# ash-shar/Long-Tail-GAN

Measured on AMD Instinct MI355X. Metric: train users/sec at BATCH_SIZE=100, higher is better.
Workload: dtype bf16

## Files before the change

### long-tail-gan_amd/csrc/ltg_fast_gen.h

```cpp
#pragma once


typedef LtgRg<1, 2, 1, 1, 4> Rg16x32;
typedef LtgRg<1, 2, 1, 1, 8> Rg16x32k8;
struct LtgRaw2 {
    ltg_f32x4 x, y;
};
constexpr int ENC1_NT = 512;
template <bool PRE>
__global__ __launch_bounds__(ENC1_NT) void fk_enc1(int B, int H, int Z, const float* __restrict__ h1, const float* __restrict__ Wq1,
                                              const float* __restrict__ bq1, const float* __restrict__ eps_in, float is_training,
                                              uint64_t seed, uint64_t step, float* __restrict__ mulv, float* __restrict__ z,
                                              const float* __restrict__ bq0 = nullptr, float* __restrict__ h1_out = nullptr,
                                              LtgGate end_wait = LTG_NO_GATE) {
    LTG_STAMP_AT(11, 0);
    __shared__ __attribute__((aligned(16))) float lds[Rg16x32k8::LDS_FLOATS];
    const LtgTile2 tl = xcd_tile2();
    const int m0 = tl.y * 16, n0 = tl.x * 16, Z2 = 2 * Z;
    auto col = [=] __device__(int c) { return min(n0 + (c & 15), Z - 1) + (c >> 4) * Z; };
    auto a_ld = [=] __device__(int, int m, int k) {
        if constexpr (PRE) return LtgRaw2{ltg_ld4(h1 + (size_t)m * H + k), ltg_ld4(bq0 + k)};
        else return ltg_ld4(h1 + (size_t)m * H + k);
    };
    const bool keep_h1 = PRE && tl.x == 0;
// ... 123 lines not shown
                                            float anneal, uint64_t seed, uint64_t step, float* __restrict__ dmlv) {
    LTG_STAMP_AT(15, 0);
    __shared__ __attribute__((aligned(16))) float lds[Rg16::LDS_FLOATS];
    const LtgTile2 tl = xcd_tile2();
    dz_tile(B, Z, H, da2, Wp0, mulv, eps_in, is_training, anneal, seed, step, dmlv, tl.y * 16, tl.x * 16, lds);
}
__global__ __launch_bounds__(NT) void fk_dz_dh2(int B, int Z, int H, const float* __restrict__ dh2, const float* __restrict__ h2,
                                                const float* __restrict__ Wp0, const float* __restrict__ mulv, const float* __restrict__ eps_in,
                                                float is_training, float anneal, uint64_t seed, uint64_t step, float* __restrict__ dmlv,
                                                float* __restrict__ da2_out) {
    __shared__ __attribute__((aligned(16))) float lds[Rg16::LDS_FLOATS];
    const LtgTile2 tl = xcd_tile2();
    dz_tile<true>(B, Z, H, dh2, Wp0, mulv, eps_in, is_training, anneal, seed, step, dmlv, tl.y * 16, tl.x * 16, lds, h2, da2_out, tl.x == 0);
}
__global__ __launch_bounds__(NT) void fk_dh1(int B, int H, int Z2, const float* __restrict__ dmlv, const float* __restrict__ Wq1,
                                             const float* __restrict__ h1, float* __restrict__ da1) {
    LTG_STAMP_AT(16, 0);
    __shared__ __attribute__((aligned(16))) float lds[Rg16::LDS_FLOATS];
    const LtgTile2 tl = xcd_tile2();
    dh1_tile(B, H, Z2, dmlv, Wq1, h1, da1, tl.y * 16, tl.x * 16, lds);
}

constexpr int E0_U = 8;
__global__ __launch_bounds__(ENC_NT) void fk_enc0_fwd(int H, int I, const int32_t* __restrict__ indptr, const int32_t* __restrict__ indices,
                                                      const float* __restrict__ values, const uint8_t* __restrict__ drop_keep, float keep,
                                                      uint64_t seed, uint64_t step, const float* __restrict__ Wq0,
                                                      const float* __restrict__ bq0, float* __restrict__ h1, float* __restrict__ row_scale,
                                                      const float* __restrict__ row_norm2, int item_lo, int Ig, int pre_only,
                                                      float* __restrict__ xd, int rps, LtgGate started = LTG_NO_GATE, LtgGate end_wait = LTG_NO_GATE) {
    if (end_wait.word && blockIdx.y == gridDim.y - 1) {
        if (blockIdx.x == 0 && threadIdx.x == 0) ltg_gate_wait_tail(end_wait);
        return;
    }
    if (blockIdx.x == 0 && blockIdx.y == 0 && threadIdx.x == 0) ltg_gate_set(started);
    extern __shared__ __attribute__((aligned(16))) float s_row[];
    __shared__ __attribute__((aligned(16))) float4 s_part[ENC_NW][64];
    __shared__ int s_idx[ENC_NT];
    __shared__ float s_val[ENC_NT];
    __shared__ float red[ENC_NW];
    const int b = blockIdx.y, cb = blockIdx.x, tid = threadIdx.x, lane = tid & 63, w = tid >> 6;
    const uint64_t kb = rps > 0 ? (uint64_t)(b % rps) : (uint64_t)b;
    step += rps > 0 ? (uint64_t)(b / rps) : 0;
    const int beg = indptr[b], end = indptr[b + 1];
    float4 bb = make_float4(0.f, 0.f, 0.f, 0.f);
    if (!pre_only && tid < 64 && 64 * cb + tid < (H >> 2)) bb = *reinterpret_cast<const float4*>(bq0 + 4 * (64 * cb + tid));
    float ss = 0.f;
    for (int e = beg + tid; e < end; e += ENC_NT) {
        const float v = values ? values[e] : 1.f;
        ss += v * v;
    }
#pragma unroll
    for (int o = 32; o > 0; o >>= 1) ss += __shfl_xor(ss, o);
    if (lane == 0) red[w] = ss;
    __syncthreads();
    ss = 0.f;
#pragma unroll
    for (int i = 0; i < ENC_NW; ++i) ss += red[i];
    if (row_norm2) ss = row_norm2[b];
    const float scale = 1.f / (keep * sqrtf(fmaxf(ss, 1e-12f)));
    if (tid == 0 && cb == 0) row_scale[b] = scale;
    const int H4 = H >> 2;
    const int c4 = min(64 * cb + lane, H4 - 1);
    const bool dense = xd != nullptr && cb == 0;
// ... 314 lines not shown
```

### long-tail-gan_amd/csrc/ltg_fast_small.h

```cpp
#pragma once


template <bool BF>
__global__ __launch_bounds__(NT) void fk_dec1(int B, int I, int H, const float* __restrict__ h2, const float* __restrict__ Wp1t,
                                              const float* __restrict__ bp1, float* __restrict__ logits) {
    __shared__ __attribute__((aligned(16))) float lds[Rg16::LDS_FLOATS];
    const LtgTile2 tl = xcd_tile2();
    const int m0 = tl.y * 16, n0 = tl.x * 16;
    auto a_ld = [=] __device__(int, int m, int k) { return ltg_ld4(h2 + (size_t)m * H + k); };
    auto b_ld = [=] __device__(int, int k, int n) { return ltg_ld4(Wp1t + (size_t)n * H + k); };
    auto xf = [=] __device__(ltg_f32x4 v, int, int, int) { return BF ? ltg_bf16r4(v) : v; };
    const float biasv = bp1[min(n0 + (int)(threadIdx.x & 15), I - 1)];
    auto epi = [=] __device__(int, int m, int n, float v, bool ok) {
        if (ok) logits[(size_t)m * I + n] = v + biasv;
    };
    if constexpr (BF) ltg_rgemm<1, 1, 1, 1, 4, 5, true>(B, I, H, m0, n0, a_ld, xf, b_ld, xf, epi, lds);
    else ltg_rgemm<1, 1, 1, 1, 4, 10>(B, I, H, m0, n0, a_ld, xf, b_ld, xf, epi, lds);
}

__device__ __forceinline__ void block_red4(float& a, float& b, float& c, float& mx, float (*red)[NT / 64]) {
#pragma unroll
    for (int o = 32; o > 0; o >>= 1) {
        a += __shfl_xor(a, o);
        b += __shfl_xor(b, o);
// ... 120 lines not shown
    const float l = mx + logf(s);
    const float ps = psu / s;
    const float invB = 1.f / (float)B, invs = 1.f / s;
    const float c = cntv > 0 ? lam / (float)cntv * sy : 0.f;
    const float alpha = nx * invB + c * ps;
#pragma unroll
    for (int j = 0; j < PER; ++j) {
        const int i = tid + NT * j;
        if (i < I) {
            const float p = expf(v[j] - mx) * invs;
            dlog[(size_t)b * I + i] = p * alpha - s_x[i] * invB - (s_s[i] ? c * p : 0.f);
        }
    }
    if (tid == 0) {
        lse[b] = l;
        float* o = rowout + (size_t)b * 4;
        o[0] = -xl + nx * l;
        o[1] = ps;
        o[2] = klb;
        o[3] = sy;
    }
}

constexpr int DH2_NT = 512;
template <bool BF>
__global__ __launch_bounds__(DH2_NT) void fk_dh2(int B, int I, int H, const float* __restrict__ dlog, const float* __restrict__ Wp1t,
                                             const float* __restrict__ h2, float* __restrict__ da2) {
    __shared__ __attribute__((aligned(16))) float lds[LtgRg<1, 1, 1, 1, 8>::LDS_FLOATS];
    const LtgTile2 tl = xcd_tile2();
    const int m0 = tl.y * 16, n0 = tl.x * 16;
    auto a_ld = [=] __device__(int, int m, int k) { return ltg_ld4(dlog + (size_t)m * I + k); };
    auto b_ld = [=] __device__(int, int k, int n) { return ltg_ld4s(Wp1t + (size_t)k * H + n, H); };
    auto xf = [=] __device__(ltg_f32x4 v, int, int, int) { return BF ? ltg_bf16r4(v) : v; };
    const float t = h2[(size_t)min(m0 + (int)(threadIdx.x >> 4), B - 1) * H + min(n0 + (int)(threadIdx.x & 15), H - 1)];
    auto epi = [=] __device__(int, int m, int n, float v, bool ok) {
        if (ok) da2[(size_t)m * H + n] = v * (1.f - t * t);
    };
    if constexpr (BF) ltg_rgemm<1, 1, 1, 1, 8, 4, true>(B, H, I, m0, n0, a_ld, xf, b_ld, xf, epi, lds);
    else ltg_rgemm<1, 1, 1, 1, 8, 8>(B, H, I, m0, n0, a_ld, xf, b_ld, xf, epi, lds);
}

struct WgTensors {
    float *W, *mW, *vW, *b, *mb, *vb;
};
struct WgWhere {
    float *p, *m, *v;
    bool vec;
};
struct WgRegs {
    ltg_f32x4 p, m, v;
};
#ifndef LTG_TAIL_BN
#define LTG_TAIL_BN 32
#endif
template <bool RND, bool ONES_L>
__device__ __forceinline__ void wgrad_adam_tile(int K, int Min, int Nin, const float* __restrict__ Lm, int ldl, const float* __restrict__ Rm,
                                                int ldr, WgTensors T, int ldw, AdamC ad, int m0, int n0, float* __restrict__ lds, unsigned dead = 0u) {
    const int M = ONES_L ? Min + 1 : Min, N = ONES_L ? Nin : Nin + 1;
    auto a_ld = [=] __device__(int, int m, int k) {
        ltg_f32x4 v;
#pragma unroll
// ... 225 lines not shown
```

### long-tail-gan_amd/csrc/ltg_gemm.h

```cpp
#pragma once
#include <hip/hip_runtime.h>
#include <stdint.h>

typedef __attribute__((ext_vector_type(4))) float ltg_f32x4;
typedef __attribute__((ext_vector_type(8))) __bf16 ltg_bf16x8;
typedef __attribute__((ext_vector_type(8))) unsigned short ltg_u16x8;

__device__ __forceinline__ unsigned short ltg_f2bf(float x) {
    unsigned u = __float_as_uint(x);
    u += 0x7FFFu + ((u >> 16) & 1u);
    return (unsigned short)(u >> 16);
}

__device__ __forceinline__ unsigned char ltg_f2fp8(float x) {
    const float c = fminf(fmaxf(x, -448.f), 448.f);
    return (unsigned char)(__builtin_amdgcn_cvt_pk_fp8_f32(c, 0.f, 0, false) & 0xFF);
}

template <int MODE, int BK_> struct LtgGemmCfg;
template <int BK_> struct LtgGemmCfg<1, BK_> {
    typedef unsigned short T;
    static constexpr int BK = BK_;
    static constexpr int LDK = BK_ + 8;
    static_assert(BK_ % 32 == 0, "bf16 K-step is 32");
// ... 214 lines not shown
                for (int r = 0; r < 4; ++r)
                    Cs[(wm * WTM + i * 16 + lq * 4 + r) * LDC + wn * WTN + j * 16 + lr] = acc[i][j][r];
        __syncthreads();
        constexpr int N4 = BN / 4;
#pragma unroll
        for (int e = tid; e < BM * N4; e += NT) {
            const int mm = e / N4, c4 = e % N4;
            const int m = m0 + mm, n = n0 + c4 * 4;
            if (m < M && n < N) epi(m, n, *reinterpret_cast<const float4*>(&Cs[mm * LDC + c4 * 4]));
        }
    } else {
#pragma unroll
        for (int i = 0; i < TM; ++i)
#pragma unroll
            for (int j = 0; j < TN; ++j)
#pragma unroll
                for (int r = 0; r < 4; ++r) {
                    const int m = m0 + wm * WTM + i * 16 + lq * 4 + r;
                    const int n = n0 + wn * WTN + j * 16 + lr;
                    if (m < M && n < N) epi(m, n, acc[i][j][r]);
                }
    }
}
```

### long-tail-gan_amd/csrc/ltg_kernels.hip

```cpp
#include <hip/hip_runtime.h>
#include <math.h>
#include <stdint.h>

#include "../../include/ltg.h"
#include "ltg_gemm.h"
#include "ltg_rng.h"

namespace {

constexpr int NT = 256;

struct AdamC {
    float lr_t, b1, b2, eps;
};

__device__ __forceinline__ float adam_move(const float p, const float lm, const float v, const float eps) {
#ifdef LTG_ADAM_IEEE
    return p - lm / (sqrtf(v) + eps);
#else
    return __builtin_fmaf(-lm, __builtin_amdgcn_rcpf(__builtin_amdgcn_sqrtf(v) + eps), p);
#endif
}
__device__ __forceinline__ void adam1(float& p, float& m, float& v, const float g, const float lr_t, const AdamC& c) {
    m = __builtin_fmaf(c.b1, m, (1.f - c.b1) * g);
// ... 121 lines not shown
    return c < 4 * ST_BN ? 4 * ST_BN : c;
}

inline int dh2_kchunk(int I) {
    int chunk = (I + 63) / 64;
    chunk = (chunk + 31) / 32 * 32;
    if (chunk < 256) chunk = 256;
    return chunk;
}

inline size_t gq0_rows(const ltg_config* cfg, int ) { return (size_t)cfg->n_items; }

constexpr int RD_MAXI = 4096;
struct Workspace {
    float *rowpart, *segpart, *nb, *Pb, *scal, *dlog, *part, *dh2, *da2, *dmlv, *da1, *gq0;
    int32_t* slotmap;
    float *A1, *A3, *y, *ds, *lrow, *dpre1, *dpre3, *slab;
    float *spart, *G3, *rowout, *xd;
    uint8_t* A1_8;
    uint8_t *A1T_8, *dpre3_8, *dpre3T_8, *dpre1T_8, *ET_8;
    unsigned short* dA1T_16;
    int np8;
    float* wsp;
    size_t bytes;
};
inline int d_slab_stride(int P) { return (P + 1 + 3) & ~3; }

constexpr int FT_BM = 64, FT_NT = 512;
constexpr int FT_KP1_MAX = 4;
inline int ft_lda(int h12) { return ((h12 + 31) & ~31) + 4; }
inline size_t ft_lds_bytes(int h12) { return ((size_t)FT_BM * ft_lda(h12) + 4 * FT_BM) * sizeof(float); }
inline size_t ft_wsp_triples(int h0, int h1, int h2, int h3) {
    const size_t kp1 = (h0 + 31) / 32, kp3 = (h1 + h2 + 31) / 32;
    return (size_t)((h1 + 15) / 16) * kp1 + (size_t)((h2 + 15) / 16) * kp1 + (size_t)((h3 + 15) / 16) * kp3;
}
inline size_t ft_wsp_bytes(int h0, int h1, int h2, int h3) { return ft_wsp_triples(h0, h1, h2, h3) * 3 * 1024; }
inline bool ft_wsp_capable(const ltg_config* c) {
    return (c->tuning & 262144) == 0 && c->d_precision == LTG_PREC_FP32 && !(c->d_h0 >= 512 && c->d_h1 + c->d_h2 >= 512 && c->d_h3 >= 128) && c->d_h0 >= 4 &&
           c->d_h0 <= 32 * FT_KP1_MAX && (c->d_h0 % 4) == 0 && c->d_h1 >= 1 && c->d_h2 >= 1 && c->d_h3 >= 1 && c->d_h3 <= 320 &&
           ft_lds_bytes(c->d_h1 + c->d_h2) <= (size_t)160 * 1024;
}
Workspace carve(const ltg_config* cfg, int max_rows, int max_pairs, char* base) {
    Workspace w;
    size_t off = 0;
    auto take = [&](size_t nfloat) {
        float* p = reinterpret_cast<float*>(base + off);
        off += align_up(nfloat * sizeof(float));
        return p;
    };
    const size_t R = (size_t)max_rows, I = (size_t)cfg->n_items, H = (size_t)cfg->h_enc, Z = (size_t)cfg->z_dim;
    const size_t P = (size_t)max_pairs, h12 = (size_t)cfg->d_h1 + cfg->d_h2, h3 = (size_t)cfg->d_h3;
    const int kchunk = dh2_kchunk(cfg->n_items);
    size_t nsplit = (I + kchunk - 1) / kchunk;
    {
        const size_t ns2 = (I + dh2_stream_chunk(cfg->n_items) - 1) / dh2_stream_chunk(cfg->n_items);
        if (ns2 > nsplit) nsplit = ns2;
    }
    w.rowpart = take(R * RP);
    w.segpart = take(segpart_floats(I, R));
    w.nb = take(R);
    w.Pb = take(R);
    w.scal = take(16);
    w.dlog = take(R * I);
// ... 14 lines not shown
    {
        const DLayout L = d_layout(cfg->d_h0, cfg->d_h1, cfg->d_h2, cfg->d_h3);
        const size_t ks = (P + D_KCHUNK - 1) / D_KCHUNK;
        w.slab = take(ks * (size_t)d_slab_stride(L.off[8]));
    }
    w.spart = take((((h3 + 31) / 32) + 1) * P);
    w.G3 = take(P * h3);
    w.rowout = take(R * 4);
    w.xd = take(I <= (size_t)RD_MAXI ? R * I : 1);
    w.A1_8 = reinterpret_cast<uint8_t*>(take((P * h12 + 3) / 4));
    {
        const bool f8 = cfg->d_precision == LTG_PREC_FP8;
        const size_t np = ((P + 127) / 128 * 128), h0 = (size_t)cfg->d_h0;
        auto take8 = [&](size_t nbytes) { return reinterpret_cast<uint8_t*>(take(f8 ? (nbytes + 3) / 4 : 1)); };
        w.np8 = (int)np;
        w.A1T_8 = take8((h12 + 1) * np);
        w.dA1T_16 = reinterpret_cast<unsigned short*>(take8(2 * h12 * np));
        w.dpre3_8 = take8(P * h3);
        w.dpre3T_8 = take8(h3 * np);
        w.dpre1T_8 = take8(h12 * np);
        w.ET_8 = take8(2 * (h0 + 1) * np);
    }
    w.wsp = take(ft_wsp_capable(cfg) ? ft_wsp_bytes(cfg->d_h0, cfg->d_h1, cfg->d_h2, cfg->d_h3) / sizeof(float) : 1);
    w.bytes = off;
    return w;
}

inline AdamC make_adam(const ltg_config* cfg, int t) {
    AdamC a;
    const double b1 = cfg->beta1, b2 = cfg->beta2;
    a.lr_t = (float)((double)cfg->lr * sqrt(1.0 - pow(b2, (double)t)) / (1.0 - pow(b1, (double)t)));
    a.b1 = cfg->beta1;
    a.b2 = cfg->beta2;
    a.eps = cfg->adam_eps;
    return a;
}

struct Probe {
    const ltg_probe* p;
    hipStream_t st;
    inline void before(int id) const {
        if (p && p->kernel_id == id && p->ev_start) (void)hipEventRecord((hipEvent_t)p->ev_start, st);
    }
    inline void after(int id) const {
        if (p && p->kernel_id == id && p->ev_stop) (void)hipEventRecord((hipEvent_t)p->ev_stop, st);
    }
// ... 29 lines not shown
}
inline bool d_fast(const ltg_config* c) {
    return fast_on(c) && c->d_precision == LTG_PREC_FP32 && !d_wide(c) && c->d_h3 <= 512 && (c->d_h0 % 4) == 0 && ((c->d_h1 + c->d_h2) % 4) == 0 && (c->d_h3 % 4) == 0;
}
#ifndef LTG_D_SPLIT_SET
#define LTG_D_SPLIT_SET 0xE
#endif
inline int d_spl(const ltg_config* c, int which) {
    const int mode = c->d_arith & 3, set = ((c->d_arith >> 4) & 15) ? ((c->d_arith >> 4) & 15) : (mode == LTG_DARITH_BF16X4 ? 0xF : LTG_D_SPLIT_SET);
    if (mode == LTG_DARITH_FP32 || !((set >> which) & 1)) return 0;
    return mode == LTG_DARITH_BF16X4 ? 4 : 6;
}
#define LTG_D_SPL_LAUNCH(SPLV, KERNEL, ...)                                       \
    do {                                                                          \
        if ((SPLV) == 6) hipLaunchKernelGGL((KERNEL<6>), __VA_ARGS__);            \
        else if ((SPLV) == 4) hipLaunchKernelGGL((KERNEL<4>), __VA_ARGS__);       \
        else hipLaunchKernelGGL((KERNEL<0>), __VA_ARGS__);                        \
    } while (0)
inline bool unsharded(const ltg_config* c) { return c->item_lo == 0 && (c->n_items_global == 0 || c->n_items_global == c->n_items); }
inline bool small_fast(const ltg_config* c, int rows) {
    return fast_on(c) && unsharded(c) && c->n_items <= RD_MAXI && (c->n_items % 4) == 0 && (c->z_dim % 4) == 0 && rows <= 256;
}

constexpr int32_t TUNING_BITS = (1 << 14) | (1 << 17) | (1 << 18) | (1 << 19) | (1 << 20) | (1 << 21) | (1 << 22) | (1 << 26);
bool cfg_ok(const ltg_config* c) {
    return c && c->n_items > 0 && c->h_enc > 0 && c->h_enc <= 768 && (c->h_enc % 4) == 0 && c->z_dim > 0 &&
           c->d_h0 >= 1 && c->d_h1 >= 1 && c->d_h2 >= 1 && c->d_h3 >= 1 &&
           (c->precision == LTG_PREC_BF16 || c->precision == LTG_PREC_FP32) && c->d_precision >= 0 && c->d_precision <= LTG_PREC_FP8 &&
           c->d_arith >= 0 && (c->d_arith & 3) <= LTG_DARITH_BF16X4 && (c->d_arith & ~0xF3) == 0 && (c->tuning & ~TUNING_BITS) == 0;
}

inline int Ig_of(const ltg_config* cfg) { return cfg->n_items_global > 0 ? cfg->n_items_global : cfg->n_items; }

inline bool q0_lazy(const ltg_config* cfg, const ltg_gen_state* gen) {
    return gen->q0_last && gen->q0_lr_hist && gen->q0_period >= 1 && gen->q0_period <= LTG_Q0_HIST / 2 && gen->q0_ord >= 0 && (cfg->h_enc % 4) == 0 &&
           cfg->n_items >= 8192;
}
void q0_touch(const ltg_config* cfg, const ltg_gen_state* gen, const ltg_batch* bt, hipStream_t st, const unsigned* poison = nullptr,
              int32_t* mark = nullptr, unsigned seq = 0u) {
    if (!q0_lazy(cfg, gen) || bt->n_rows <= 0) return;
    const AdamC ad = make_adam(cfg, 1);
    if (bt->uptr && bt->csr_pos) {
        if (bt->n_unique > 0)
            hipLaunchKernelGGL(k_q0_touch_unique, dim3(bt->n_unique), dim3(Q0_NT), 0, st, cfg->h_enc, bt->n_unique, bt->uptr, bt->csr_pos, bt->indices, bt->uitem,
                               gen->q0_ord, *gen, ad, poison, mark, seq);
    } else {
        hipLaunchKernelGGL(k_q0_touch_rows, dim3(bt->n_rows), dim3(Q0_NT), 0, st, cfg->h_enc, bt->n_rows, bt->indptr, bt->indices, gen->q0_ord, *gen, ad);
    }
}

void fwd_stage_enc(const ltg_config* cfg, const ltg_gen_state* gen, const ltg_batch* bt, const ltg_fwd_opts* o,
                   const ltg_gen_acts* acts, int pre_only, hipStream_t st, float* xd = nullptr, bool touched = false,
                   LtgGate started = LTG_NO_GATE, LtgGate end_wait = LTG_NO_GATE) {
    const int R = bt->n_rows, I = cfg->n_items, H = cfg->h_enc;
    const Probe pr{o->probe, st};
    if (!touched) q0_touch(cfg, gen, bt, st);
    if (fast_on(cfg)) {
        LTG_PROBED(pr, LTG_K_ENC0_FWD,
                   hipLaunchKernelGGL(fk_enc0_fwd, dim3((H / 4 + 63) / 64, R + (end_wait.word ? 1 : 0)), dim3(ENC_NT), xd ? (size_t)I * sizeof(float) : 0, st, H, I, bt->indptr,
                                      bt->indices, bt->values, o->drop_keep, o->keep_prob, cfg->seed, o->rng_step, gen->p[0], gen->p[4], acts->h1,
                                      acts->row_scale, bt->row_norm2, cfg->item_lo, Ig_of(cfg), pre_only, xd, o->rows_per_step, started, end_wait));
        return;
    }
    LTG_PROBED(pr, LTG_K_ENC0_FWD,
               hipLaunchKernelGGL(k_enc0_fwd, dim3(R), dim3(ENC_NT), (size_t)ENC_NW * H * sizeof(float), st, H, I, bt->indptr, bt->indices,
                                  bt->values, o->drop_keep, o->keep_prob, cfg->seed, o->rng_step, gen->p[0], gen->p[4], acts->h1,
                                  acts->row_scale, bt->row_norm2, cfg->item_lo, Ig_of(cfg), pre_only, o->rows_per_step));
}

int launch_dec1_fwd_stream(const ltg_config* cfg, const ltg_gen_state* gen, int R, const ltg_gen_acts* acts, float* stat, hipStream_t st) {
    const int I = cfg->n_items, H = cfg->h_enc;
    const int st2_min = (cfg->tuning & (1 << 17)) ? 8192 : ST2_MIN_ITEMS;
    if ((cfg->tuning & (1 << 26)) == 0 && I >= st2_min && (size_t)R * (size_t)I < ((size_t)1 << 30) &&
        (size_t)I * (size_t)(ST_KP * 2) < ((size_t)1 << 32)) {
        const int nt2 = (I + 31) / 32, G2 = nt2 < 256 ? nt2 : 256;
#define LTG_ST2(STATS, NTB) hipLaunchKernelGGL((k_dec1_fwd_stream2<STATS, NTB>), dim3(G2), dim3(ST_NT), (size_t)ST_KS * NTB * 64 * 16, st, R, I, H, acts->h2, gen->wp1t_bf16, gen->p[7], acts->logits, stat)
        if (stat) { if (R <= 112) LTG_ST2(true, 7); else LTG_ST2(true, 8); }
        else { if (R <= 112) LTG_ST2(false, 7); else LTG_ST2(false, 8); }
#undef LTG_ST2
        return G2;
    }
    const int ntiles = (I + ST_BN - 1) / ST_BN, G = ntiles < 256 ? ntiles : 256;
// ... 705 lines not shown
    if (ltg_workspace_bytes(cfg, B, nf) > ws_bytes) return LTG_EWORKSPACE;
    hipStream_t st = (hipStream_t)stream;
    Workspace w = carve(cfg, B, nf, (char*)ws);
    const bool have_y = o->y_pre != nullptr;
    if (have_y) w.y = const_cast<float*>(o->y_pre);
    q0_touch(cfg, gen, bt, st);
    const bool aux_sweep = q0_lazy(cfg, gen) && o->aux_stream && o->ev_fork && o->ev_sweep;
    const bool fork = o->aux_stream && o->ev_fork && o->ev_join && nf > 0 && !have_y;
    if (fork || aux_sweep) {
        hipStream_t aux = (hipStream_t)o->aux_stream;
        if (hipEventRecord((hipEvent_t)o->ev_fork, st) != hipSuccess || hipStreamWaitEvent(aux, (hipEvent_t)o->ev_fork, 0) != hipSuccess)
            return LTG_ELAUNCH;
        if (fork) {
            PairView pv{0, nf, nullptr, nullptr, fake->pop, fake->niche};
            DropView dA{nullptr, o->drop_fake[0], 0, 0}, dB{nullptr, o->drop_fake[1], 0, 0}, dC{nullptr, o->drop_fake[2], 0, 0};
            disc_forward(cfg, disc, pv, dA, dB, dC, o->d_keep_prob, o->d_rng_step, w, false, nullptr, aux);
            if (hipEventRecord((hipEvent_t)o->ev_join, aux) != hipSuccess) return LTG_ELAUNCH;
        }
    }
    ltg_g_opts o_local = *o;
    o_local.fake_done = (o->fake_done & 1) | (aux_sweep ? G_AUX_SWEEP : 0);
    o = &o_local;
    const bool small = small_fast(cfg, B);
    fwd_stage_enc(cfg, gen, bt, &o->fwd, acts, 0, st, small ? w.xd : nullptr, true);
    const int sgroups = fwd_stage_rest(cfg, gen, bt, &o->fwd, acts, 0, st, small ? nullptr : w.segpart);
    if (small) {
        const int I = cfg->n_items, H = cfg->h_enc;
        const Probe pr{o->probe, st};
        if (nf > 0 && !fork && !have_y) {
            PairView pv{0, nf, nullptr, nullptr, fake->pop, fake->niche};
            DropView dA{nullptr, o->drop_fake[0], 0, 0}, dB{nullptr, o->drop_fake[1], 0, 0}, dC{nullptr, o->drop_fake[2], 0, 0};
            disc_forward(cfg, disc, pv, dA, dB, dC, o->d_keep_prob, o->d_rng_step, w, false, o->probe, st);
        }
        if (fork && hipStreamWaitEvent(st, (hipEvent_t)o->ev_join, 0) != hipSuccess) return LTG_ELAUNCH;
        LTG_PROBED(pr, LTG_K_ROW_DLOGITS, hipLaunchKernelGGL(fk_row_dlogits, dim3(B), dim3(NT), 0, st, B, I, bt->indptr, bt->indices, bt->values, acts->logits,
                                                             acts->kl_rows, w.y, nf, o->cnt, o->gan_lambda, fake->row, fake->niche, fake->pop, w.dlog,
                                                             acts->lse, w.rowout));
        pr.before(LTG_K_DH2);
        if (cfg->precision == LTG_PREC_BF16) hipLaunchKernelGGL(fk_dh2<true>, grid2(H, B, 16, 16), dim3(DH2_NT), 0, st, B, I, H, w.dlog, gen->p[3], acts->h2, w.da2);
        else hipLaunchKernelGGL(fk_dh2<false>, grid2(H, B, 16, 16), dim3(DH2_NT), 0, st, B, I, H, w.dlog, gen->p[3], acts->h2, w.da2);
        pr.after(LTG_K_DH2);
        g_chain(cfg, gen, bt, o, acts, w, make_adam(cfg, o->adam_t), nullptr, true, loss_out, st);
        return check_launch();
    }
    g_row_partial(cfg, bt, fake, acts, w.rowpart, st, w.segpart, nullptr, sgroups);
    if (fork && hipStreamWaitEvent(st, (hipEvent_t)o->ev_join, 0) != hipSuccess) return LTG_ELAUNCH;
    int rc = g_stage_bwd_dec(cfg, gen, disc, bt, fake, o, acts, w.rowpart, 1, loss_out, w, w.da2, st, fork || have_y, acts->h2);
    if (rc != LTG_OK) return rc;
    rc = g_stage_bwd_rest(cfg, gen, bt, o, acts, w.da2, w, st, true);
    if (aux_sweep && hipStreamWaitEvent(st, (hipEvent_t)o->ev_sweep, 0) != hipSuccess) return LTG_ELAUNCH;
    return rc;
}

int ltg_g_fwd_enc(const ltg_config* cfg, const ltg_gen_state* gen, const ltg_batch* bt, const ltg_fwd_opts* opts,
                  const ltg_gen_acts* acts, ltg_stream stream) {
    clear_errors();
    if (!g_args_ok(cfg, gen, bt, acts) || !opts) return LTG_EINVAL;
    fwd_stage_enc(cfg, gen, bt, opts, acts, 1, (hipStream_t)stream);
    return check_launch();
}

int ltg_g_fwd_rest(const ltg_config* cfg, const ltg_gen_state* gen, const ltg_batch* bt, const ltg_pairs* fake,
// ... 641 lines not shown
```

### long-tail-gan_amd/csrc/ltg_rgemm.h

```cpp
#pragma once
#include <hip/hip_runtime.h>
#include <stdint.h>

#include "ltg_gemm.h"

__device__ __forceinline__ ltg_f32x4 ltg_ld4(const float* __restrict__ p) { return *reinterpret_cast<const ltg_f32x4*>(p); }
__device__ __forceinline__ ltg_f32x4 ltg_ld4s(const float* __restrict__ p, size_t s) { return ltg_f32x4{p[0], p[s], p[2 * s], p[3 * s]}; }
__device__ __forceinline__ float ltg_bf16r(float x) { return __uint_as_float((unsigned)ltg_f2bf(x) << 16); }
__device__ __forceinline__ ltg_f32x4 ltg_bf16r4(ltg_f32x4 v) { return ltg_f32x4{ltg_bf16r(v[0]), ltg_bf16r(v[1]), ltg_bf16r(v[2]), ltg_bf16r(v[3])}; }

#ifdef LTG_STAMP
__device__ unsigned long long ltg_stamp_buf[16384 * 8];
__device__ __forceinline__ void ltg_stamp(int slot) {
    if (threadIdx.x == 0) {
        const unsigned wg = blockIdx.x + gridDim.x * (blockIdx.y + gridDim.y * blockIdx.z);
        if (wg < 16384u)
            ltg_stamp_buf[wg * 8 + slot] = slot == 6 ? ((unsigned long long)__builtin_amdgcn_s_getreg((4 << 0) | (0 << 6) | (31 << 11)) |
                                                        ((unsigned long long)__builtin_amdgcn_s_getreg((20 << 0) | (0 << 6) | (31 << 11)) << 32))
                                                     : wall_clock64();
    }
}
#define LTG_STAMP_AT(SID, slot) do { if constexpr ((SID) == LTG_STAMP) ltg_stamp(slot); } while (0)
#else
#define LTG_STAMP_AT(SID, slot) do { } while (0)
// ... 176 lines not shown
                    for (int tn = 0; tn < TN; ++tn)
                        acc[tm][tn] = __builtin_amdgcn_mfma_f32_16x16x4f32(av[tm][j], bv[tn][j], acc[tm][tn], 0, 0, 0);
        }
    };
    if constexpr (PEEL) {
        pass(0);
        for (int base = NBLK; base < per; base += NBLK) pass(base);
    } else {
        for (int base = 0; base < per; base += NBLK) pass(base);
    }
    LTG_STAMP_AT(SID, 3);
    float* mine = lds + wk * (G::BM * G::LDC);
#pragma unroll
    for (int tm = 0; tm < TM; ++tm)
#pragma unroll
        for (int tn = 0; tn < TN; ++tn)
#pragma unroll
            for (int x = 0; x < 4; ++x)
                mine[((wm * TM + tm) * 16 + 4 * q + x) * G::LDC + (wn * TN + tn) * 16 + r] = acc[tm][tn][x];
    __syncthreads();
    LTG_STAMP_AT(SID, 4);
}

template <int TM, int TN, int WM, int WN, int WK, int NBLK, bool PEEL = false, class ALD, class AXF, class BLD, class BXF, class MID = LtgNoMid>
__device__ __forceinline__ void ltg_rgemm_product_bf16(int M, int N, int K, int m0, int n0, ALD a_ld, AXF a_xf, BLD b_ld, BXF b_xf, float* __restrict__ lds,
                                                       MID mid = MID()) {
    static_assert(WM * WN * WK == 4 || WM * WN * WK == 8, "4 or 8 waves per workgroup");
    typedef LtgRg<TM, TN, WM, WN, WK> G;
    const int tid = threadIdx.x, lane = tid & 63, w = tid >> 6;
    const int r = lane & 15, q = lane >> 4;
    const int wk = w % WK, wn = (w / WK) % WN, wm = w / (WK * WN);
    const int nblk = (K + 31) >> 5;
    const int per = (nblk + WK - 1) / WK;
    const int Kc = K >= 4 ? ((K - 1) & ~3) : 0;
    int am[TM], bn[TN];
    bool aok[TM];
#pragma unroll
    for (int tm = 0; tm < TM; ++tm) {
        const int m = m0 + (wm * TM + tm) * 16 + r;
        aok[tm] = m < M;
        am[tm] = min(m, M - 1);
    }
#pragma unroll
    for (int tn = 0; tn < TN; ++tn) bn[tn] = min(n0 + (wn * TN + tn) * 16 + r, N - 1);
    ltg_f32x4 acc[TM][TN];
#pragma unroll
    for (int tm = 0; tm < TM; ++tm)
#pragma unroll
        for (int tn = 0; tn < TN; ++tn) acc[tm][tn] = ltg_f32x4{0.f, 0.f, 0.f, 0.f};
    auto pack8 = [] __device__(ltg_f32x4 lo, ltg_f32x4 hi) -> ltg_bf16x8 {
        typedef unsigned ltg_rg_u32x4 __attribute__((ext_vector_type(4)));
        ltg_rg_u32x4 p;
        p[0] = (__float_as_uint(lo[0]) >> 16) | (__float_as_uint(lo[1]) & 0xFFFF0000u);
        p[1] = (__float_as_uint(lo[2]) >> 16) | (__float_as_uint(lo[3]) & 0xFFFF0000u);
        p[2] = (__float_as_uint(hi[0]) >> 16) | (__float_as_uint(hi[1]) & 0xFFFF0000u);
        p[3] = (__float_as_uint(hi[2]) >> 16) | (__float_as_uint(hi[3]) & 0xFFFF0000u);
        return __builtin_bit_cast(ltg_bf16x8, p);
    };
    auto pass = [&] __device__(const int base) {
        decltype(a_ld(0, 0, 0)) ra[NBLK][TM][2];
        decltype(b_ld(0, 0, 0)) rb[NBLK][TN][2];
#pragma unroll
        for (int i = 0; i < NBLK; ++i) {
#pragma unroll
            for (int h = 0; h < 2; ++h) {
                const int kc = min(32 * (wk * per + base + i) + 8 * q + 4 * h, Kc);
#pragma unroll
                for (int tm = 0; tm < TM; ++tm) ra[i][tm][h] = a_ld(2 * i + h, am[tm], kc);
#pragma unroll
                for (int tn = 0; tn < TN; ++tn) rb[i][tn][h] = b_ld(2 * i + h, kc, bn[tn]);
            }
        }
        __builtin_amdgcn_sched_barrier(0);
        if (base == 0) mid();
#pragma unroll
        for (int i = 0; i < NBLK; ++i) {
            if (base + i >= per || 32 * (wk * per + base + i) >= K) continue;
            ltg_f32x4 av[TM][2], bv[TN][2];
#pragma unroll
            for (int h = 0; h < 2; ++h) {
                const int k = 32 * (wk * per + base + i) + 8 * q + 4 * h;
                const bool ok = k < K;
                const int kc = min(k, Kc);
#pragma unroll
                for (int tm = 0; tm < TM; ++tm) {
                    const ltg_f32x4 v = a_xf(ra[i][tm][h], 2 * i + h, am[tm], kc);
                    const bool o = ok && aok[tm];
                    av[tm][h] = ltg_f32x4{o ? v[0] : 0.f, o ? v[1] : 0.f, o ? v[2] : 0.f, o ? v[3] : 0.f};
                }
#pragma unroll
                for (int tn = 0; tn < TN; ++tn) bv[tn][h] = b_xf(rb[i][tn][h], 2 * i + h, kc, bn[tn]);
            }
            ltg_bf16x8 ap[TM], bp[TN];
#pragma unroll
            for (int tm = 0; tm < TM; ++tm) ap[tm] = pack8(av[tm][0], av[tm][1]);
#pragma unroll
            for (int tn = 0; tn < TN; ++tn) bp[tn] = pack8(bv[tn][0], bv[tn][1]);
#pragma unroll
            for (int tm = 0; tm < TM; ++tm)
#pragma unroll
                for (int tn = 0; tn < TN; ++tn) acc[tm][tn] = __builtin_amdgcn_mfma_f32_16x16x32_bf16(ap[tm], bp[tn], acc[tm][tn], 0, 0, 0);
        }
    };
    if constexpr (PEEL) {
        pass(0);
        for (int base = NBLK; base < per; base += NBLK) pass(base);
    } else {
        for (int base = 0; base < per; base += NBLK) pass(base);
    }
    float* mine = lds + wk * (G::BM * G::LDC);
#pragma unroll
    for (int tm = 0; tm < TM; ++tm)
#pragma unroll
        for (int tn = 0; tn < TN; ++tn)
#pragma unroll
            for (int x = 0; x < 4; ++x)
                mine[((wm * TM + tm) * 16 + 4 * q + x) * G::LDC + (wn * TN + tn) * 16 + r] = acc[tm][tn][x];
    __syncthreads();
}

template <int TM, int TN, int WM, int WN, int WK, int NBLK, bool BFM = false, bool PEEL = false, int SID = 0, int SPL = 0, class ALD, class AXF, class BLD, class BXF, class EF, class MID = LtgNoMid>
__device__ __forceinline__ void ltg_rgemm(int M, int N, int K, int m0, int n0, ALD a_ld, AXF a_xf, BLD b_ld, BXF b_xf, EF epi, float* __restrict__ lds,
                                          MID mid = MID()) {
    typedef LtgRg<TM, TN, WM, WN, WK> G;
    static_assert(!(BFM && SPL != 0), "operands that are bf16-rounded anyway need no split");
    if constexpr (BFM) ltg_rgemm_product_bf16<TM, TN, WM, WN, WK, NBLK, PEEL>(M, N, K, m0, n0, a_ld, a_xf, b_ld, b_xf, lds, mid);
    else
    ltg_rgemm_product<TM, TN, WM, WN, WK, NBLK, PEEL, SID, SPL>(M, N, K, m0, n0, a_ld, a_xf, b_ld, b_xf, lds, mid);
    const int tid = threadIdx.x;
    constexpr int NE = G::BM * G::BN;
    constexpr int NTH = 64 * WM * WN * WK;
    static_assert(NE % NTH == 0 || (NE < NTH && NE % 64 == 0), "tile must divide over the workgroup's threads, or be finished by its first waves");
    if (NE < NTH && tid >= NE) return;
#pragma unroll
    for (int e = 0; e < (NE + NTH - 1) / NTH; ++e) {
        const int id = tid + NTH * e;
        const int mm = id / G::BN, nn = id % G::BN;
        float v = lds[mm * G::LDC + nn];
#pragma unroll
        for (int s = 1; s < WK; ++s) v += lds[s * (G::BM * G::LDC) + mm * G::LDC + nn];
        const int m = m0 + mm, n = n0 + nn;
        epi(e, m, n, v, m < M && n < N);
    }
    LTG_STAMP_AT(SID, 5);
    LTG_STAMP_AT(SID, 6);
}

template <int TM, int TN, int WM, int WN, int WK, int NBLK, bool BFM = false, int SPL = 0, class ALD, class AXF, class BLD, class BXF, class PF, class EF>
__device__ __forceinline__ void ltg_rgemm_v4(int M, int N, int K, int m0, int n0, ALD a_ld, AXF a_xf, BLD b_ld, BXF b_xf, PF prefetch, EF epi4,
// ... 29 lines not shown
```

Measured before the change: 87060.

## Prebuild bf16 MFMA-ready image of Wp1t in enc0 kernel for dh2 GEMM

Adds extra workgroups to the encoder-0 forward kernel that convert the decoder weight Wp1t into a packed bf16 image laid out in the exact per-lane order the MFMA loop consumes. The dh2 backward GEMM then loads one 16-byte vector per block instead of strided fp32 loads followed by rounding and packing. This aims to remove the strided transposed weight reads and per-use conversion from the backward pass. In exchange it uses extra workspace, lengthens the enc0 launch, and can be turned off with tuning bit 8.

```diff
diff --git a/long-tail-gan_amd/csrc/ltg_fast_gen.h b/long-tail-gan_amd/csrc/ltg_fast_gen.h
--- a/long-tail-gan_amd/csrc/ltg_fast_gen.h
+++ b/long-tail-gan_amd/csrc/ltg_fast_gen.h
@@ -169,23 +169,38 @@
 }
 
 constexpr int E0_U = 8;
+struct GImgJob {
+    ltg_rg_u32x4* img;
+    const float* Wp1t;
+    int rows;
+};
+template <bool IMG = false>
 __global__ __launch_bounds__(ENC_NT) void fk_enc0_fwd(int H, int I, const int32_t* __restrict__ indptr, const int32_t* __restrict__ indices,
                                                       const float* __restrict__ values, const uint8_t* __restrict__ drop_keep, float keep,
                                                       uint64_t seed, uint64_t step, const float* __restrict__ Wq0,
                                                       const float* __restrict__ bq0, float* __restrict__ h1, float* __restrict__ row_scale,
                                                       const float* __restrict__ row_norm2, int item_lo, int Ig, int pre_only,
-                                                      float* __restrict__ xd, int rps, LtgGate started = LTG_NO_GATE, LtgGate end_wait = LTG_NO_GATE) {
+                                                      float* __restrict__ xd, int rps, LtgGate started = LTG_NO_GATE, LtgGate end_wait = LTG_NO_GATE,
+                                                      GImgJob wimg = GImgJob{nullptr, nullptr, 0}) {
     if (end_wait.word && blockIdx.y == gridDim.y - 1) {
         if (blockIdx.x == 0 && threadIdx.x == 0) ltg_gate_wait_tail(end_wait);
         return;
     }
     if (blockIdx.x == 0 && blockIdx.y == 0 && threadIdx.x == 0) ltg_gate_set(started);
+    if constexpr (IMG) {
+        if ((int)blockIdx.y < wimg.rows) {
+            const int nbs = ltg_bimg16_blocks(I, DH2_WK, DH2_NBLK);
+            const int wv = (blockIdx.y * gridDim.x + blockIdx.x) * ENC_NW + (threadIdx.x >> 6);
+            if (wv < ((H + 15) / 16) * DH2_WK * nbs) ltg_bimg16_build<DH2_WK, DH2_NBLK>(H, I, wimg.Wp1t, (size_t)H, wimg.img, wv / (DH2_WK * nbs), (wv / nbs) % DH2_WK, wv % nbs);
+            return;
+        }
+    }
     extern __shared__ __attribute__((aligned(16))) float s_row[];
     __shared__ __attribute__((aligned(16))) float4 s_part[ENC_NW][64];
     __shared__ int s_idx[ENC_NT];
     __shared__ float s_val[ENC_NT];
     __shared__ float red[ENC_NW];
-    const int b = blockIdx.y, cb = blockIdx.x, tid = threadIdx.x, lane = tid & 63, w = tid >> 6;
+    const int b = (int)blockIdx.y - (IMG ? wimg.rows : 0), cb = blockIdx.x, tid = threadIdx.x, lane = tid & 63, w = tid >> 6;
     const uint64_t kb = rps > 0 ? (uint64_t)(b % rps) : (uint64_t)b;
     step += rps > 0 ? (uint64_t)(b / rps) : 0;
     const int beg = indptr[b], end = indptr[b + 1];
diff --git a/long-tail-gan_amd/csrc/ltg_fast_small.h b/long-tail-gan_amd/csrc/ltg_fast_small.h
--- a/long-tail-gan_amd/csrc/ltg_fast_small.h
+++ b/long-tail-gan_amd/csrc/ltg_fast_small.h
@@ -166,10 +166,10 @@
     }
 }
 
-constexpr int DH2_NT = 512;
-template <bool BF>
+template <bool BF, bool IMG = false>
 __global__ __launch_bounds__(DH2_NT) void fk_dh2(int B, int I, int H, const float* __restrict__ dlog, const float* __restrict__ Wp1t,
-                                             const float* __restrict__ h2, float* __restrict__ da2) {
+                                             const float* __restrict__ h2, float* __restrict__ da2, const ltg_rg_u32x4* __restrict__ wimg = nullptr) {
+    static_assert(!IMG || BF, "the image holds bf16");
     __shared__ __attribute__((aligned(16))) float lds[LtgRg<1, 1, 1, 1, 8>::LDS_FLOATS];
     const LtgTile2 tl = xcd_tile2();
     const int m0 = tl.y * 16, n0 = tl.x * 16;
@@ -180,7 +180,11 @@
     auto epi = [=] __device__(int, int m, int n, float v, bool ok) {
         if (ok) da2[(size_t)m * H + n] = v * (1.f - t * t);
     };
-    if constexpr (BF) ltg_rgemm<1, 1, 1, 1, 8, 4, true>(B, H, I, m0, n0, a_ld, xf, b_ld, xf, epi, lds);
+    if constexpr (IMG) {
+        const int nbs = ltg_bimg16_blocks(I, DH2_WK, DH2_NBLK);
+        auto b_img = [=] __device__(int blk, int wk, int ct) { return ltg_bimg16_ld(wimg, ct, DH2_WK, wk, nbs, blk); };
+        ltg_rgemm<1, 1, 1, 1, DH2_WK, DH2_NBLK, true, false, 0, 0, true>(B, H, I, m0, n0, a_ld, xf, b_img, xf, epi, lds);
+    } else if constexpr (BF) ltg_rgemm<1, 1, 1, 1, DH2_WK, DH2_NBLK, true>(B, H, I, m0, n0, a_ld, xf, b_ld, xf, epi, lds);
     else ltg_rgemm<1, 1, 1, 1, 8, 8>(B, H, I, m0, n0, a_ld, xf, b_ld, xf, epi, lds);
 }
 
diff --git a/long-tail-gan_amd/csrc/ltg_gemm.h b/long-tail-gan_amd/csrc/ltg_gemm.h
--- a/long-tail-gan_amd/csrc/ltg_gemm.h
+++ b/long-tail-gan_amd/csrc/ltg_gemm.h
@@ -260,3 +260,7 @@
                 }
     }
 }
+
+__host__ __device__ inline int ltg_rg_per32(int K, int WK) { return (((K + 31) >> 5) + WK - 1) / WK; }
+__host__ __device__ inline int ltg_bimg16_blocks(int K, int WK, int NBLK) { return (ltg_rg_per32(K, WK) + NBLK - 1) / NBLK * NBLK; }
+__host__ __device__ inline size_t ltg_bimg16_entries(int N, int K, int WK, int NBLK) { return (size_t)((N + 15) / 16) * WK * ltg_bimg16_blocks(K, WK, NBLK) * 64; }
diff --git a/long-tail-gan_amd/csrc/ltg_kernels.hip b/long-tail-gan_amd/csrc/ltg_kernels.hip
--- a/long-tail-gan_amd/csrc/ltg_kernels.hip
+++ b/long-tail-gan_amd/csrc/ltg_kernels.hip
@@ -167,6 +167,7 @@
     unsigned short* dA1T_16;
     int np8;
     float* wsp;
+    float* wp1img;
     size_t bytes;
 };
 inline int d_slab_stride(int P) { return (P + 1 + 3) & ~3; }
@@ -184,6 +185,11 @@
     return (c->tuning & 262144) == 0 && c->d_precision == LTG_PREC_FP32 && !(c->d_h0 >= 512 && c->d_h1 + c->d_h2 >= 512 && c->d_h3 >= 128) && c->d_h0 >= 4 &&
            c->d_h0 <= 32 * FT_KP1_MAX && (c->d_h0 % 4) == 0 && c->d_h1 >= 1 && c->d_h2 >= 1 && c->d_h3 >= 1 && c->d_h3 <= 320 &&
            ft_lds_bytes(c->d_h1 + c->d_h2) <= (size_t)160 * 1024;
+}
+constexpr int DH2_NT = 512, DH2_WK = 8, DH2_NBLK = 4;
+inline bool g_img_capable(const ltg_config* c) {
+    return (c->tuning & 262144) == 0 && c->item_lo == 0 && (c->n_items_global == 0 || c->n_items_global == c->n_items) && c->n_items <= RD_MAXI &&
+           (c->n_items % 4) == 0 && (c->z_dim % 4) == 0 && c->precision == LTG_PREC_BF16;
 }
 Workspace carve(const ltg_config* cfg, int max_rows, int max_pairs, char* base) {
     Workspace w;
@@ -244,6 +250,7 @@
         w.ET_8 = take8(2 * (h0 + 1) * np);
     }
     w.wsp = take(ft_wsp_capable(cfg) ? ft_wsp_bytes(cfg->d_h0, cfg->d_h1, cfg->d_h2, cfg->d_h3) / sizeof(float) : 1);
+    w.wp1img = take(g_img_capable(cfg) ? ltg_bimg16_entries((int)H, (int)I, DH2_WK, DH2_NBLK) * 4 : 1);
     w.bytes = off;
     return w;
 }
@@ -319,7 +326,7 @@
     return fast_on(c) && unsharded(c) && c->n_items <= RD_MAXI && (c->n_items % 4) == 0 && (c->z_dim % 4) == 0 && rows <= 256;
 }
 
-constexpr int32_t TUNING_BITS = (1 << 14) | (1 << 17) | (1 << 18) | (1 << 19) | (1 << 20) | (1 << 21) | (1 << 22) | (1 << 26);
+constexpr int32_t TUNING_BITS = (1 << 8) | (1 << 14) | (1 << 17) | (1 << 18) | (1 << 19) | (1 << 20) | (1 << 21) | (1 << 22) | (1 << 26);
 bool cfg_ok(const ltg_config* c) {
     return c && c->n_items > 0 && c->h_enc > 0 && c->h_enc <= 768 && (c->h_enc % 4) == 0 && c->z_dim > 0 &&
            c->d_h0 >= 1 && c->d_h1 >= 1 && c->d_h2 >= 1 && c->d_h3 >= 1 &&
@@ -348,13 +355,22 @@
 
 void fwd_stage_enc(const ltg_config* cfg, const ltg_gen_state* gen, const ltg_batch* bt, const ltg_fwd_opts* o,
                    const ltg_gen_acts* acts, int pre_only, hipStream_t st, float* xd = nullptr, bool touched = false,
-                   LtgGate started = LTG_NO_GATE, LtgGate end_wait = LTG_NO_GATE) {
+                   LtgGate started = LTG_NO_GATE, LtgGate end_wait = LTG_NO_GATE, float* wp1img = nullptr) {
     const int R = bt->n_rows, I = cfg->n_items, H = cfg->h_enc;
     const Probe pr{o->probe, st};
     if (!touched) q0_touch(cfg, gen, bt, st);
+    if (fast_on(cfg) && wp1img) {
+        const int gx = (H / 4 + 63) / 64, nwv = ((H + 15) / 16) * DH2_WK * ltg_bimg16_blocks(I, DH2_WK, DH2_NBLK);
+        const GImgJob ij{reinterpret_cast<ltg_rg_u32x4*>(wp1img), gen->p[3], (nwv + gx * ENC_NW - 1) / (gx * ENC_NW)};
+        LTG_PROBED(pr, LTG_K_ENC0_FWD,
+                   hipLaunchKernelGGL(fk_enc0_fwd<true>, dim3(gx, R + ij.rows + (end_wait.word ? 1 : 0)), dim3(ENC_NT), xd ? (size_t)I * sizeof(float) : 0, st, H, I, bt->indptr,
+                                      bt->indices, bt->values, o->drop_keep, o->keep_prob, cfg->seed, o->rng_step, gen->p[0], gen->p[4], acts->h1,
+                                      acts->row_scale, bt->row_norm2, cfg->item_lo, Ig_of(cfg), pre_only, xd, o->rows_per_step, started, end_wait, ij));
+        return;
+    }
     if (fast_on(cfg)) {
         LTG_PROBED(pr, LTG_K_ENC0_FWD,
-                   hipLaunchKernelGGL(fk_enc0_fwd, dim3((H / 4 + 63) / 64, R + (end_wait.word ? 1 : 0)), dim3(ENC_NT), xd ? (size_t)I * sizeof(float) : 0, st, H, I, bt->indptr,
+                   hipLaunchKernelGGL(fk_enc0_fwd<false>, dim3((H / 4 + 63) / 64, R + (end_wait.word ? 1 : 0)), dim3(ENC_NT), xd ? (size_t)I * sizeof(float) : 0, st, H, I, bt->indptr,
                                       bt->indices, bt->values, o->drop_keep, o->keep_prob, cfg->seed, o->rng_step, gen->p[0], gen->p[4], acts->h1,
                                       acts->row_scale, bt->row_norm2, cfg->item_lo, Ig_of(cfg), pre_only, xd, o->rows_per_step, started, end_wait));
         return;
@@ -1106,7 +1122,8 @@
     o_local.fake_done = (o->fake_done & 1) | (aux_sweep ? G_AUX_SWEEP : 0);
     o = &o_local;
     const bool small = small_fast(cfg, B);
-    fwd_stage_enc(cfg, gen, bt, &o->fwd, acts, 0, st, small ? w.xd : nullptr, true);
+    const bool wimg = small && g_img_capable(cfg) && (cfg->tuning & (1 << 8)) == 0;
+    fwd_stage_enc(cfg, gen, bt, &o->fwd, acts, 0, st, small ? w.xd : nullptr, true, LTG_NO_GATE, LTG_NO_GATE, wimg ? w.wp1img : nullptr);
     const int sgroups = fwd_stage_rest(cfg, gen, bt, &o->fwd, acts, 0, st, small ? nullptr : w.segpart);
     if (small) {
         const int I = cfg->n_items, H = cfg->h_enc;
@@ -1121,7 +1138,9 @@
                                                              acts->kl_rows, w.y, nf, o->cnt, o->gan_lambda, fake->row, fake->niche, fake->pop, w.dlog,
                                                              acts->lse, w.rowout));
         pr.before(LTG_K_DH2);
-        if (cfg->precision == LTG_PREC_BF16) hipLaunchKernelGGL(fk_dh2<true>, grid2(H, B, 16, 16), dim3(DH2_NT), 0, st, B, I, H, w.dlog, gen->p[3], acts->h2, w.da2);
+        if (wimg) hipLaunchKernelGGL((fk_dh2<true, true>), grid2(H, B, 16, 16), dim3(DH2_NT), 0, st, B, I, H, w.dlog, gen->p[3], acts->h2, w.da2,
+                                     reinterpret_cast<const ltg_rg_u32x4*>(w.wp1img));
+        else if (cfg->precision == LTG_PREC_BF16) hipLaunchKernelGGL(fk_dh2<true>, grid2(H, B, 16, 16), dim3(DH2_NT), 0, st, B, I, H, w.dlog, gen->p[3], acts->h2, w.da2);
         else hipLaunchKernelGGL(fk_dh2<false>, grid2(H, B, 16, 16), dim3(DH2_NT), 0, st, B, I, H, w.dlog, gen->p[3], acts->h2, w.da2);
         pr.after(LTG_K_DH2);
         g_chain(cfg, gen, bt, o, acts, w, make_adam(cfg, o->adam_t), nullptr, true, loss_out, st);
diff --git a/long-tail-gan_amd/csrc/ltg_rgemm.h b/long-tail-gan_amd/csrc/ltg_rgemm.h
--- a/long-tail-gan_amd/csrc/ltg_rgemm.h
+++ b/long-tail-gan_amd/csrc/ltg_rgemm.h
@@ -222,7 +222,35 @@
     LTG_STAMP_AT(SID, 4);
 }
 
-template <int TM, int TN, int WM, int WN, int WK, int NBLK, bool PEEL = false, class ALD, class AXF, class BLD, class BXF, class MID = LtgNoMid>
+typedef unsigned ltg_rg_u32x4 __attribute__((ext_vector_type(4)));
+__device__ __forceinline__ ltg_rg_u32x4 ltg_pack8(ltg_f32x4 lo, ltg_f32x4 hi) {
+    ltg_rg_u32x4 p;
+    p[0] = (__float_as_uint(lo[0]) >> 16) | (__float_as_uint(lo[1]) & 0xFFFF0000u);
+    p[1] = (__float_as_uint(lo[2]) >> 16) | (__float_as_uint(lo[3]) & 0xFFFF0000u);
+    p[2] = (__float_as_uint(hi[0]) >> 16) | (__float_as_uint(hi[1]) & 0xFFFF0000u);
+    p[3] = (__float_as_uint(hi[2]) >> 16) | (__float_as_uint(hi[3]) & 0xFFFF0000u);
+    return p;
+}
+__device__ __forceinline__ int ltg_rg_kc32(int K, int per, int wk, int blk, int q, int h) { return min(32 * (wk * per + blk) + 8 * q + 4 * h, K >= 4 ? ((K - 1) & ~3) : 0); }
+__device__ __forceinline__ size_t ltg_bimg16_at(int ct, int WK, int wk, int nbs, int blk, int lane) { return (size_t)((ct * WK + wk) * nbs + blk) * 64 + lane; }
+__device__ __forceinline__ ltg_rg_u32x4 ltg_bimg16_ld(const ltg_rg_u32x4* __restrict__ img, int ct, int WK, int wk, int nbs, int blk) {
+    return img[ltg_bimg16_at(ct, WK, wk, nbs, blk, threadIdx.x & 63)];
+}
+template <int WK, int NBLK>
+__device__ __forceinline__ void ltg_bimg16_build(int N, int K, const float* __restrict__ B, size_t sk, ltg_rg_u32x4* __restrict__ img, int ct, int wk, int blk) {
+    const int lane = threadIdx.x & 63, r = lane & 15, q = lane >> 4;
+    const int per = ltg_rg_per32(K, WK);
+    const float* col = B + min(16 * ct + r, N - 1);
+    ltg_f32x4 x[2];
+#pragma unroll
+    for (int h = 0; h < 2; ++h) {
+        const float* p = col + (size_t)ltg_rg_kc32(K, per, wk, blk, q, h) * sk;
+        x[h] = ltg_f32x4{p[0], p[sk], p[2 * sk], p[3 * sk]};
+    }
+    img[ltg_bimg16_at(ct, WK, wk, ltg_bimg16_blocks(K, WK, NBLK), blk, lane)] = ltg_pack8(ltg_bf16r4(x[0]), ltg_bf16r4(x[1]));
+}
+
+template <int TM, int TN, int WM, int WN, int WK, int NBLK, bool PEEL = false, bool BIMG = false, class ALD, class AXF, class BLD, class BXF, class MID = LtgNoMid>
 __device__ __forceinline__ void ltg_rgemm_product_bf16(int M, int N, int K, int m0, int n0, ALD a_ld, AXF a_xf, BLD b_ld, BXF b_xf, float* __restrict__ lds,
                                                        MID mid = MID()) {
     static_assert(WM * WN * WK == 4 || WM * WN * WK == 8, "4 or 8 waves per workgroup");
@@ -248,18 +276,10 @@
     for (int tm = 0; tm < TM; ++tm)
 #pragma unroll
         for (int tn = 0; tn < TN; ++tn) acc[tm][tn] = ltg_f32x4{0.f, 0.f, 0.f, 0.f};
-    auto pack8 = [] __device__(ltg_f32x4 lo, ltg_f32x4 hi) -> ltg_bf16x8 {
-        typedef unsigned ltg_rg_u32x4 __attribute__((ext_vector_type(4)));
-        ltg_rg_u32x4 p;
-        p[0] = (__float_as_uint(lo[0]) >> 16) | (__float_as_uint(lo[1]) & 0xFFFF0000u);
-        p[1] = (__float_as_uint(lo[2]) >> 16) | (__float_as_uint(lo[3]) & 0xFFFF0000u);
-        p[2] = (__float_as_uint(hi[0]) >> 16) | (__float_as_uint(hi[1]) & 0xFFFF0000u);
-        p[3] = (__float_as_uint(hi[2]) >> 16) | (__float_as_uint(hi[3]) & 0xFFFF0000u);
-        return __builtin_bit_cast(ltg_bf16x8, p);
-    };
+    auto pack8 = [] __device__(ltg_f32x4 lo, ltg_f32x4 hi) -> ltg_bf16x8 { return __builtin_bit_cast(ltg_bf16x8, ltg_pack8(lo, hi)); };
     auto pass = [&] __device__(const int base) {
         decltype(a_ld(0, 0, 0)) ra[NBLK][TM][2];
-        decltype(b_ld(0, 0, 0)) rb[NBLK][TN][2];
+        decltype(b_ld(0, 0, 0)) rb[NBLK][TN][BIMG ? 1 : 2];
 #pragma unroll
         for (int i = 0; i < NBLK; ++i) {
 #pragma unroll
@@ -267,8 +287,15 @@
                 const int kc = min(32 * (wk * per + base + i) + 8 * q + 4 * h, Kc);
 #pragma unroll
                 for (int tm = 0; tm < TM; ++tm) ra[i][tm][h] = a_ld(2 * i + h, am[tm], kc);
-#pragma unroll
-                for (int tn = 0; tn < TN; ++tn) rb[i][tn][h] = b_ld(2 * i + h, kc, bn[tn]);
+                if constexpr (BIMG) {
+                    if (h == 0) {
+#pragma unroll
+                        for (int tn = 0; tn < TN; ++tn) rb[i][tn][0] = b_ld(base + i, wk, (n0 >> 4) + wn * TN + tn);
+                    }
+                } else {
+#pragma unroll
+                    for (int tn = 0; tn < TN; ++tn) rb[i][tn][h] = b_ld(2 * i + h, kc, bn[tn]);
+                }
             }
         }
         __builtin_amdgcn_sched_barrier(0);
@@ -288,14 +315,19 @@
                     const bool o = ok && aok[tm];
                     av[tm][h] = ltg_f32x4{o ? v[0] : 0.f, o ? v[1] : 0.f, o ? v[2] : 0.f, o ? v[3] : 0.f};
                 }
-#pragma unroll
-                for (int tn = 0; tn < TN; ++tn) bv[tn][h] = b_xf(rb[i][tn][h], 2 * i + h, kc, bn[tn]);
+                if constexpr (!BIMG) {
+#pragma unroll
+                    for (int tn = 0; tn < TN; ++tn) bv[tn][h] = b_xf(rb[i][tn][h], 2 * i + h, kc, bn[tn]);
+                }
             }
             ltg_bf16x8 ap[TM], bp[TN];
 #pragma unroll
             for (int tm = 0; tm < TM; ++tm) ap[tm] = pack8(av[tm][0], av[tm][1]);
 #pragma unroll
-            for (int tn = 0; tn < TN; ++tn) bp[tn] = pack8(bv[tn][0], bv[tn][1]);
+            for (int tn = 0; tn < TN; ++tn) {
+                if constexpr (BIMG) bp[tn] = __builtin_bit_cast(ltg_bf16x8, rb[i][tn][0]);
+                else bp[tn] = pack8(bv[tn][0], bv[tn][1]);
+            }
 #pragma unroll
             for (int tm = 0; tm < TM; ++tm)
 #pragma unroll
@@ -319,12 +351,13 @@
     __syncthreads();
 }
 
-template <int TM, int TN, int WM, int WN, int WK, int NBLK, bool BFM = false, bool PEEL = false, int SID = 0, int SPL = 0, class ALD, class AXF, class BLD, class BXF, class EF, class MID = LtgNoMid>
+template <int TM, int TN, int WM, int WN, int WK, int NBLK, bool BFM = false, bool PEEL = false, int SID = 0, int SPL = 0, bool BIMG = false, class ALD, class AXF, class BLD, class BXF, class EF, class MID = LtgNoMid>
 __device__ __forceinline__ void ltg_rgemm(int M, int N, int K, int m0, int n0, ALD a_ld, AXF a_xf, BLD b_ld, BXF b_xf, EF epi, float* __restrict__ lds,
                                           MID mid = MID()) {
     typedef LtgRg<TM, TN, WM, WN, WK> G;
     static_assert(!(BFM && SPL != 0), "operands that are bf16-rounded anyway need no split");
-    if constexpr (BFM) ltg_rgemm_product_bf16<TM, TN, WM, WN, WK, NBLK, PEEL>(M, N, K, m0, n0, a_ld, a_xf, b_ld, b_xf, lds, mid);
+    static_assert(BFM || !BIMG, "operand images exist for the bf16 product");
+    if constexpr (BFM) ltg_rgemm_product_bf16<TM, TN, WM, WN, WK, NBLK, PEEL, BIMG>(M, N, K, m0, n0, a_ld, a_xf, b_ld, b_xf, lds, mid);
     else
     ltg_rgemm_product<TM, TN, WM, WN, WK, NBLK, PEEL, SID, SPL>(M, N, K, m0, n0, a_ld, a_xf, b_ld, b_xf, lds, mid);
     const int tid = threadIdx.x;
```

Result: faster. 88140, median of 6 (+1.2%).
